# Freebirdgo/MapReduce_Rust

Measured on AMD Instinct MI355X. Metric: word-count input GB/s (whole node) at 1/2/4/8 MI355X + % of HBM roofline, higher is better.
Workload: dtype u8

## Files before the change

### mapreduce_rust_amd/csrc/k_keys.hip

```cpp
#include <algorithm>
#include <type_traits>

#include "mrg_device.h"
#include "mrg_internal.h"

namespace {

inline dim3 grid_for(uint64_t n, int b = 256) { return dim3((unsigned)((n + b - 1) / b)); }

template <int WG>
__device__ __forceinline__ uint64_t wg_append(unsigned long long *counter, bool pred, uint32_t *s_w,
                                              unsigned long long *s_base) {
    const uint64_t m = __ballot(pred);
    const uint32_t wv = threadIdx.x >> 6, lane = __lane_id();
    if (lane == 0) s_w[wv] = (uint32_t)__popcll(m);
    __syncthreads();
    if (threadIdx.x == 0) {
        uint32_t run = 0;
        for (int w = 0; w < WG / 64; ++w) {
            const uint32_t c = s_w[w];
            s_w[w] = run;
            run += c;
        }
        *s_base = run ? atomicAdd(counter, (unsigned long long)run) : 0ull;
// ... 387 lines not shown
    const uint64_t kbase = s_base;
    for (int pp = 0; pp < NP; ++pp) {
        const int i = min(pp * BA_WG + tid, (int)BA_CAP - 1);
        const BaKey k = s_key[i];
        const bool full = pp * BA_WG + tid < (int)BA_CAP && k.a != MRG_EMPTY_K0;
        const uint64_t m = __ballot(full);
        const uint64_t j = kbase + s_po[pp * BA_NW + wv] + (uint64_t)__popcll(m & mrg_lanemask_lt());
        if (full && j < A.kcap) {
            gk(A.out.k0)[j] = k.a;
            gk(A.out.k1)[j] = k.b;
            gk(A.out.cnt)[j] = s_cnt[i];
            gk(A.out.doc)[j] = IDX ? s_doc[i] : MRG_EMPTY_DOC;
            const uint32_t L = mrg_short_len(k.a, k.b);
            gk(A.out.len)[j] = L;
            gk(A.out.hoff)[j] = MRG_NO_HEAP;
            if (A.n_reduce) gk(A.out.part)[j] = (uint32_t)(mrg_siphash_short(k.a, k.b, L) % (uint64_t)A.n_reduce);
        }
    }
}

__global__ __launch_bounds__(1024) void k_stage_scatter(const uint8_t *stage, uint32_t table_off, uint32_t nops) {
    const StageOp *ops = reinterpret_cast<const StageOp *>(stage + table_off);
    for (uint32_t k = 0; k < nops; ++k) {
        const StageOp op = ops[k];
        uint8_t *dst = reinterpret_cast<uint8_t *>(op.dst);
        const bool fill = op.src == 0xFFFFFFFFu;
        if (((op.dst | op.n) & 3u) == 0u) {
            const uint32_t f4 = op.fill * 0x01010101u;
            const uint32_t *src = reinterpret_cast<const uint32_t *>(stage + (fill ? 0u : op.src));
            for (uint32_t i = threadIdx.x; i < op.n / 4u; i += blockDim.x)
                reinterpret_cast<uint32_t *>(dst)[i] = fill ? f4 : src[i];
// ... 354 lines not shown
    r.a = ks.k0[i];
    r.b = ks.k1[i];
    if (idx) {
        r.v = ks.doc[i];
        out[slot] = r;
        return;
    }
    for (uint64_t k = 0; k < nr; ++k) {
        const uint64_t c = cnt > vmax ? vmax : cnt;
        cnt -= c;
        r.v = (uint32_t)c;
        out[slot + k] = r;
    }
}

__global__ void k_make_sortrec(KeySet ks, uint64_t n, const uint32_t *doc_rank, SortRec *out, int carry) {
    const uint64_t i = (uint64_t)blockIdx.x * blockDim.x + threadIdx.x;
    if (i >= n) return;
    SortRec r;
    r.k0 = ks.k0[i];
    r.k1 = ks.k1[i];
    r.part = ks.part[i];
    r.doc = doc_rank ? doc_rank[ks.doc[i]] : 0u;
    r.idx = (uint32_t)i;
    r.pad = 0;
    if (carry) {
        const uint64_t c = ks.cnt[i];
        const uint32_t len = ks.len[i];
        r.doc = (uint32_t)c;
        r.pad = (len <= 16u ? len : 0xFFu) | ((uint32_t)(c >> 32) << 8);
    }
    out[i] = r;
// ... 76 lines not shown
}
void mrg_launch_export_count(KeySet ks, uint64_t n, uint32_t n_owners, unsigned long long *rec_cnt,
                             unsigned long long *heap_cnt, bool indexer, uint64_t vmax, hipStream_t s) {
    if (!n) return;
    hipLaunchKernelGGL(k_export_count, grid_for(n, EXP_WG), dim3(EXP_WG), 0, s, ks, n, n_owners, rec_cnt, heap_cnt,
                       indexer, vmax);
}
void mrg_launch_export_pack(KeySet ks, const uint8_t *heap, uint64_t n, uint32_t n_owners,
                            const uint64_t *rec_base, const uint64_t *heap_base, unsigned long long *rec_cur,
                            unsigned long long *heap_cur, XRec *out, uint8_t *out_heap, bool indexer, uint64_t vmax,
                            hipStream_t s) {
    if (!n) return;
    hipLaunchKernelGGL(k_export_pack, grid_for(n, EXP_WG), dim3(EXP_WG), 0, s, ks, heap, n, n_owners, rec_base,
                       heap_base, rec_cur, heap_cur, out, out_heap, indexer, vmax);
}
void mrg_launch_make_sortrec(KeySet ks, uint64_t n, const uint32_t *doc_rank, void *recs, hipStream_t s, bool carry) {
    if (!n) return;
    hipLaunchKernelGGL(k_make_sortrec, grid_for(n), dim3(256), 0, s, ks, n, doc_rank, (SortRec *)recs, carry ? 1 : 0);
}
void mrg_launch_wide_counts(const BucketArgs &a, uint64_t *cnt, uint64_t nseg, hipStream_t s) {
    hipLaunchKernelGGL(k_wide_counts, grid_for(nseg), dim3(256), 0, s, a, cnt);
}
void mrg_launch_wide_gather(const BucketArgs &a, const uint64_t *off, uint64_t nseg, uint32_t n_reduce, SortRec *out,
                            hipStream_t s) {
    hipLaunchKernelGGL(k_wide_gather, dim3((unsigned)nseg), dim3(256), 0, s, a, off, n_reduce, out);
}
void mrg_launch_wide_heads(const SortRec *r, uint64_t n, uint64_t *head, uint64_t *cv, hipStream_t s) {
    if (n) hipLaunchKernelGGL(k_wide_heads, grid_for(n), dim3(256), 0, s, r, n, head, cv);
}
void mrg_launch_wide_keys(const SortRec *r, uint64_t n, const uint64_t *head, const uint64_t *E, KeySet ks,
                          uint64_t *F, hipStream_t s) {
    if (n) hipLaunchKernelGGL(k_wide_keys, grid_for(n), dim3(256), 0, s, r, n, head, E, ks, F);
}
// ... 17 lines not shown
```

### mapreduce_rust_amd/csrc/k_map.hip

```cpp
#include "mrg_device.h"
#include "mrg_internal.h"
#include "mrg_split.h"

namespace {

constexpr int NW = MRG_MAP_WAVES;
constexpr int WG = 64 * NW;
constexpr int SEG = MRG_MAP_SEG;
constexpr int TILE = MRG_MAP_TILE;
constexpr int HALO = MRG_MAP_HALO;
constexpr int BEHIND = MRG_MAP_BEHIND;
constexpr int NSUB = MRG_MAP_NSUB;
constexpr int BLK = NSUB * TILE;
constexpr int WIN = BEHIND + TILE + HALO + 48;
constexpr int QCAP = TILE / 2 + 16;
constexpr int NMP = 64;
static_assert(TILE == 64 * SEG, "one segment per lane");
static_assert(WIN % 16 == 0, "16-byte window rows");
static_assert(NMP == TILE / SEG, "one mask pair per segment of the tile");
static_assert(16 * (1 + TILE / 16 + HALO / 16) <= WIN, "staged vectors fit the window row");
static_assert(BEHIND + (TILE - 1) + 31 + 20 <= WIN, "the 5-dword key read stays in the window row");
static_assert(BEHIND == 16 && HALO % 16 == 0 && HALO >= 64, "one 16-byte vector behind, whole halo vectors");
static_assert(QCAP >= TILE / 2 + 1, "the token queue holds every start of a tile");
static_assert(BLK == 2 * TILE && NSUB == 2, "A/B register sets hold two tiles per lane (v0, v1)");
// ... 1403 lines not shown
    lds_only_barrier();
    MRG_FT(1);
    if (tid < 64) {
        uint32_t run = 0;
        for (int b0 = 0; b0 < MRG_NBUCKET; b0 += 64) {
            const uint32_t v = s_hist[b0 + lane];
            const uint32_t inc = wave_incl_scan(v);
            s_hist[b0 + lane] = run + inc - v;
            run += lane_u32(inc, 63);
        }
        if (lane == 0) s_hist[MRG_NBUCKET] = run;
    }
    lds_only_barrier();
    MRG_FT(2);
    GAS uint32_t *foff = gp(A.foff) + (uint64_t)blockIdx.x * (MRG_NBUCKET + 1);
    for (int b = tid; b <= MRG_NBUCKET; b += WG) foff[b] = s_hist[b];
    const uint64_t reg = (uint64_t)blockIdx.x * CAP;
    for (int i = tid; i < CAP; i += WG) {
        const KeyPair k = s_key[i];
        if (k.a == MRG_EMPTY_K0) continue;
        const uint32_t d = IDX ? s_doc[i] : MRG_EMPTY_DOC;
        const uint32_t b = bucket_of(key_hash(k.a, k.b, d, A.hash_bits));
        const uint64_t pos2 = reg + s_hist[b] + s_rank[i];
        gp(A.fk0)[pos2] = k.a;
        gp(A.fk1)[pos2] = k.b;
        gp(A.fcnt)[pos2] = s_cnt[i];
        if (IDX) gp(A.fdoc)[pos2] = d;
    }
    }
    MRG_FT(3);
    uint32_t t = my_tokens, ttl = my_tail, t16 = my_tail16;
    for (int off = 32; off > 0; off >>= 1) {
        t += __shfl_down(t, off);
// ... 179 lines not shown
```

### mapreduce_rust_amd/csrc/k_sort.hip

```cpp
#include <algorithm>
#include <cstdlib>
#include <vector>

#include "mrg_device.h"
#include "mrg_internal.h"

namespace {

constexpr int BS = 256;
constexpr int IPT = 8;
constexpr int TILE = BS * IPT;

template <class T>
__device__ __forceinline__ T wave_incl_scan(T v) {
    const int lane = __lane_id();
    for (int o = 1; o < 64; o <<= 1) {
        const T u = __shfl_up(v, o);
        if (lane >= o) v += u;
    }
    return v;
}

template <class T>
__device__ __forceinline__ T block_excl_scan(T v, T *s_wave, T *total) {
// ... 196 lines not shown
    for (int q = 0; q < TR::NPASS; ++q) {
        if (!want[q]) continue;
        bool trivial = false;
        for (int d = 0; d < 256; ++d)
            if (h[q * 256 + d] == n) { trivial = true; break; }
        if (trivial) continue;
        hipLaunchKernelGGL(k_tile_hist<TR>, dim3(ntiles), dim3(BS), 0, s, a, n, q, cnt, ntiles);
        scan_rec<uint32_t>(cnt, cnt, (uint64_t)256 * ntiles, scantmp, s);
        hipLaunchKernelGGL(k_scatter<TR>, dim3(ntiles), dim3(BS), 0, s, a, b, n, q, cnt, ntiles);
        std::swap(a, b);
        if (passes_run) ++*passes_run;
    }
    return a;
}

constexpr int MSD_BITS = 20;
constexpr uint32_t MSD_NB = 1u << MSD_BITS;
constexpr int MSD_WG = 256;
constexpr uint32_t MSD_GRID = 1024;
constexpr uint32_t MSD_LCAP = 2048;
constexpr uint32_t MSD_SMALL = 64;
constexpr uint32_t MSD_SMALL_GRID = 2048;
constexpr uint32_t MSD_MAX_BIG = 16;

__device__ __forceinline__ uint32_t msd_bucket(const SortRec &r, uint32_t pbits) {
    if (pbits >= (uint32_t)MSD_BITS) return r.part >> (pbits - MSD_BITS);
    const uint32_t c0 = (uint32_t)(r.k0 >> 56), c1 = (uint32_t)(r.k0 >> 48) & 0xFFu, c2 = (uint32_t)(r.k0 >> 40) & 0xFFu;
    const uint32_t b0 = min(c0, 127u);
    const uint32_t b1 = b0 == 127u ? 127u : min(c1, 127u);
    const uint32_t b2 = b1 == 127u ? 127u : min(c2, 127u);
    const uint32_t code = (b0 << 14) | (b1 << 7) | b2;
    const uint32_t kb = MSD_BITS - pbits;
    return (r.part << kb) | (code >> (21 - kb));
}

__device__ __forceinline__ uint32_t uni_lane(uint32_t v, uint32_t j) {
    return (uint32_t)__builtin_amdgcn_readlane((int)v, (int)j);
}

__device__ __forceinline__ bool rec_less(const SortRec &a, const SortRec &b) {
    if (a.part != b.part) return a.part < b.part;
    if (a.k0 != b.k0) return a.k0 < b.k0;
    if (a.k1 != b.k1) return a.k1 < b.k1;
    if (a.doc != b.doc) return a.doc < b.doc;
    return a.idx < b.idx;
}

__global__ void k_msd_count(const SortRec *in, uint64_t n, uint32_t pbits, uint32_t *cnt, uint32_t *rank,
                            uint32_t *zero0, uint32_t *zero1, uint32_t *zero2) {
    const uint64_t i = (uint64_t)blockIdx.x * blockDim.x + threadIdx.x;
    if (i == 0) {
        *zero0 = 0;
        *zero1 = 0;
        *zero2 = 0;
    }
    if (i >= n) return;
    rank[i] = atomicAdd(&cnt[msd_bucket(in[i], pbits)], 1u);
}

__global__ void k_msd_scatter(const SortRec *in, SortRec *out, uint64_t n, uint32_t pbits, const uint32_t *off,
                              const uint32_t *rank) {
    const uint64_t i = (uint64_t)blockIdx.x * blockDim.x + threadIdx.x;
    if (i >= n) return;
    const SortRec r = in[i];
    out[off[msd_bucket(r, pbits)] + rank[i]] = r;
// ... 125 lines not shown
    void *ltmp;
};
static MsdTmp msd_tmp(void *tmp, uint64_t n) {
    MsdTmp t;
    t.cnt = (uint32_t *)tmp;
    t.off = t.cnt + (MSD_NB + 2);
    t.big = t.off + (MSD_NB + 2);
    t.list = t.big + (MSD_MAX_BIG + 2);
    t.list2 = t.list + (MSD_NB + 2);
    t.stmp = t.list2 + (MSD_NB + 2);
    t.rank = t.stmp + scan_tmp(MSD_NB + 1);
    t.ltmp = (void *)(((uintptr_t)(t.rank + n) + 255) & ~(uintptr_t)255);
    return t;
}

void mrg_msd_sort_launch(SortRec *a, SortRec *b, uint64_t n, uint32_t pbits, void *tmp, hipStream_t s,
                         uint32_t *h_nbig) {
    *h_nbig = 0;
    if (n <= 1) return;
    const MsdTmp t = msd_tmp(tmp, n);
    hipMemsetAsync(t.cnt, 0, sizeof(uint32_t) * (MSD_NB + 2), s);
    const unsigned g = (unsigned)((n + 255) / 256);
    hipLaunchKernelGGL(k_msd_count, dim3(g), dim3(256), 0, s, a, n, pbits, t.cnt, t.rank, t.big, t.list, t.list2);
    scan_rec<uint32_t>(t.cnt, t.off, MSD_NB + 1, t.stmp, s);
    hipLaunchKernelGGL(k_msd_scatter, dim3(g), dim3(256), 0, s, a, b, n, pbits, t.off, t.rank);
    uint32_t lcap = MSD_LCAP;
    if (const char *e = getenv("MRG_TEST_SORT_LCAP")) lcap = std::max<uint32_t>(1u, std::min<uint32_t>(MSD_LCAP, (uint32_t)atoi(e)));
    hipLaunchKernelGGL(k_msd_list, dim3(MSD_NB / 1024), dim3(1024), 0, s, t.off, std::min(MSD_SMALL, lcap), t.list, t.list2);
    const uint64_t nsmall = std::min<uint64_t>(n / 2, (uint64_t)MSD_SMALL_GRID * (MSD_WG / 64));
    hipLaunchKernelGGL(k_msd_leaf_small, dim3((unsigned)((nsmall + MSD_WG / 64 - 1) / (MSD_WG / 64))), dim3(MSD_WG), 0, s,
                       b, t.off, t.list);
    hipLaunchKernelGGL(k_msd_leaf, dim3(MSD_GRID), dim3(MSD_WG), 0, s, b, t.off, t.list2, lcap, t.big);
    hipMemcpyAsync(h_nbig, t.big, sizeof(uint32_t), hipMemcpyDeviceToHost, s);
}

SortRec *mrg_msd_sort_finish(SortRec *a, SortRec *b, uint64_t n, const SortPlan &plan, void *tmp, hipStream_t s,
                             uint32_t nb) {
    if (n <= 1) return a;
// ... 48 lines not shown
```

### mapreduce_rust_amd/csrc/mrg_internal.h

```cpp
#pragma once
#include <hip/hip_runtime.h>
#include <stddef.h>
#include <stdint.h>

#ifndef MRG_MAP_WAVES
#define MRG_MAP_WAVES 16
#endif
#define MRG_MAP_WG (64 * MRG_MAP_WAVES)
#define MRG_MAP_SEG 16
#define MRG_MAP_TILE (64 * MRG_MAP_SEG)
#define MRG_MAP_HALO 64
#define MRG_MAP_BEHIND 16
#define MRG_MAP_NSUB 2

#ifndef MRG_NBUCKET_LOG2
#define MRG_NBUCKET_LOG2 8
#endif
#define MRG_NBUCKET (1 << MRG_NBUCKET_LOG2)
#define MRG_BA_CAP 7680
#define MRG_TAIL_BYTES(idx) ((idx) ? 24u : 12u)

enum {
    CNT_REC = 0,
    CNT_LONG = 1,
// ... 133 lines not shown
    const uint32_t *monext;
    uint32_t mocap;
    const uint64_t *fk0, *fk1;
    const uint32_t *fcnt, *fdoc, *foff;
    uint32_t nreg, regcap;
    uint64_t *ok0, *ok1;
    uint32_t *ocnt, *odoc;
    uint64_t ocap;
    KeySet out;
    unsigned long long *counters;
    uint32_t hash_bits;
    uint32_t ablate;
    uint32_t nsub;
    uint64_t kcap;
    uint32_t n_reduce;
};
void mrg_launch_bucket_agg(const BucketArgs &a, bool indexer, bool count32, hipStream_t s);
struct SortRec;
void mrg_launch_wide_counts(const BucketArgs &a, uint64_t *cnt, uint64_t nseg, hipStream_t s);
void mrg_launch_wide_gather(const BucketArgs &a, const uint64_t *off, uint64_t nseg, uint32_t n_reduce, SortRec *out,
                            hipStream_t s);
void mrg_launch_wide_heads(const SortRec *r, uint64_t n, uint64_t *head, uint64_t *cv, hipStream_t s);
void mrg_launch_wide_keys(const SortRec *r, uint64_t n, const uint64_t *head, const uint64_t *E, KeySet ks,
                          uint64_t *F, hipStream_t s);
void mrg_launch_wide_cnt(const uint64_t *F, uint64_t runs, uint64_t n, const uint64_t *C, uint64_t ctot, KeySet ks,
                         hipStream_t s);
void mrg_launch_table_clear(const TableArgs &t, bool indexer, hipStream_t s);
void mrg_launch_table_insert(const TableArgs &t, const uint64_t *k0, const uint64_t *k1, const uint32_t *cnt32,
                             const uint32_t *doc, uint64_t n, bool indexer, hipStream_t s);
void mrg_launch_table_insert_x(const TableArgs &t, const XRec *x, uint64_t n, bool indexer, hipStream_t s);
// ... 7 lines not shown
void mrg_launch_long_emit(const uint32_t *rep, const uint64_t *cnt_in, const uint64_t *k0, const uint64_t *k1,
                          const uint32_t *flen, const uint64_t *hoff, const uint32_t *doc, uint64_t n,
                          unsigned long long *acc, KeySet out, unsigned long long *counter, bool indexer,
                          hipStream_t s);
void mrg_launch_x_split_long(const XRec *x, uint64_t n, const uint64_t *seg_rec_end, const uint64_t *seg_heap_base,
                             uint32_t n_segs, LongItems li, unsigned long long *counter, bool indexer, hipStream_t s);
void mrg_launch_l_split_long(const LRec *x, uint64_t n, const uint64_t *seg_rec_end, const uint64_t *seg_heap_base,
                             uint32_t n_segs, LongItems li, unsigned long long *counter, hipStream_t s);
void mrg_launch_export_count(KeySet ks, uint64_t n, uint32_t n_owners, unsigned long long *rec_cnt,
                             unsigned long long *heap_cnt, bool indexer, uint64_t vmax, hipStream_t s);
void mrg_launch_export_pack(KeySet ks, const uint8_t *heap, uint64_t n, uint32_t n_owners,
                            const uint64_t *rec_base, const uint64_t *heap_base, unsigned long long *rec_cur,
                            unsigned long long *heap_cur, XRec *out, uint8_t *out_heap, bool indexer, uint64_t vmax,
                            hipStream_t s);
void mrg_launch_make_sortrec(KeySet ks, uint64_t n, const uint32_t *doc_rank, void *recs, hipStream_t s,
                             bool carry = false);
void mrg_launch_fill_u32(uint32_t *p, uint32_t v, uint64_t n, hipStream_t s);
void mrg_launch_fill_u64(uint64_t *p, uint64_t v, uint64_t n, hipStream_t s);
void mrg_launch_iota_u32(uint32_t *p, uint64_t n, hipStream_t s);

uint64_t mrg_scan_tmp_elems(uint64_t n);
void mrg_scan_u64(const uint64_t *in, uint64_t *out, uint64_t n, uint64_t *tmp, hipStream_t s);
void mrg_scan_u32(const uint32_t *in, uint32_t *out, uint64_t n, uint32_t *tmp, hipStream_t s);
struct SortRec {
    uint64_t k0, k1;
    uint32_t part, doc;
    uint32_t idx, pad;
};
struct SortPlan {
    bool use_doc, use_k1, use_k0, use_part;
    uint32_t part_bytes;
    uint32_t doc_bytes;
};
uint64_t mrg_sort_tmp_bytes(uint64_t n);
SortRec *mrg_radix_sort(SortRec *recs, SortRec *alt, uint64_t n, const SortPlan &plan, void *tmp, hipStream_t s,
                        int *passes_run);
SortRec *mrg_msd_sort(SortRec *recs, SortRec *alt, uint64_t n, uint32_t pbits, const SortPlan &plan, void *tmp,
                      hipStream_t s, uint32_t *n_big, uint32_t *h_pinned);
void mrg_msd_sort_launch(SortRec *recs, SortRec *alt, uint64_t n, uint32_t pbits, void *tmp, hipStream_t s,
                         uint32_t *h_nbig);
SortRec *mrg_msd_sort_finish(SortRec *recs, SortRec *alt, uint64_t n, const SortPlan &plan, void *tmp, hipStream_t s,
                             uint32_t nb);
void mrg_radix_sort_u64(uint64_t *keys, uint32_t *vals, uint64_t *kv_tmp, uint64_t n, void *tmp, hipStream_t s);

struct FormatArgs {
    const SortRec *recs;
    uint64_t n;
    KeySet ks;
    const uint8_t *heap;
    uint64_t heap_bytes;
    uint32_t n_reduce;
    int drop_last;
    int indexer;
    int any_long;
    int carried;
// ... 185 lines not shown
```

### mapreduce_rust_amd/csrc/mrgpu.cpp

```cpp
#include <stdarg.h>
#include <stdio.h>
#include <string.h>
#include <sys/stat.h>

#include <rccl/rccl.h>

#include <fcntl.h>
#include <unistd.h>

#include <algorithm>
#include <atomic>
#include <chrono>
#include <condition_variable>
#include <map>
#include <memory>
#include <mutex>
#include <string>
#include <thread>
#include <unordered_map>
#include <vector>

#include "mrg_internal.h"
#include "mrgpu.h"

static_assert(sizeof(XRec) == MRG_XREC_BYTES, "exchange record layout (include/mrgpu.h)");

namespace {

thread_local std::string g_err;

struct MrgError {
    int code;
    std::string msg;
};

[[noreturn]] void raise(int code, const char *fmt, ...) {
    char buf[1024];
// ... 233 lines not shown
        p.put(leaf_pk);
        *this = WideRes{};
    }
};

struct Acc {
    bool on = false;
    bool dirty = false;
    bool seeded = false;
    AccTable T{};
    uint64_t n = 0;
    KeysBuf lng;
    uint64_t in_bytes = 0, tokens = 0, long_tokens = 0;
    uint32_t batches = 0, rehashes = 0;
    double ms_fold = 0.0;
};

}

struct mrg_ctx {
    int device = 0;
    hipStream_t own = nullptr, stream = nullptr;
    Pool pool;
    unsigned long long *d_cnt = nullptr;
    unsigned long long *h_cnt = nullptr;
    uint8_t *h_stage = nullptr;
    size_t stage_used = 0;
    uint8_t *d_stage = nullptr;
    std::vector<StageOp> pend;
    size_t pend_lo = 0;
// ... 28 lines not shown
    std::vector<uint64_t> exp_rec, exp_heap;
    uint64_t xrec_vmax = MRG_XREC_VMAX;
    uint8_t *d_out = nullptr;
    uint64_t out_cap = 0, out_bytes = 0;
    std::vector<uint64_t> part_off;
    bool reduced = false;
    uint8_t *d_final = nullptr;
    uint64_t final_cap = 0, final_bytes = 0;
    bool finalized = false;
    uint8_t *d_top = nullptr;
    uint64_t top_cap = 0, top_bytes = 0, top_lines = 0;
    bool topped = false;
    uint64_t top_info[8] = {};
    uint64_t top_pass_bytes[MRG_TOPK_DIGITS] = {};
    uint64_t extra_first = 0;
    mrg_stats st{};
    uint64_t enc_info[8] = {};
    double enc_ms[4] = {};
    hipEvent_t enc_ev[6] = {};
};

struct mrg_vocab {
    int device = 0;
    uint64_t n = 0, text_bytes = 0;
    void *block = nullptr;
    VocTable T{};
};

struct mrg_comm {
    ncclComm_t comm = nullptr;
// ... 80 lines not shown
    HIPCHK(hipMemcpyAsync(c->h_cnt, c->d_cnt, sizeof(unsigned long long) * CNT_N, hipMemcpyDeviceToHost, c->stream));
    sync(c);
}

void ev_rec(mrg_ctx *c, int i) {
    if (c->timing) HIPCHK(hipEventRecord(c->ev[i], c->stream));
}
double ev_ms(mrg_ctx *c, int a, int b) {
    if (!c->timing) return 0.0;
    float ms = 0;
    HIPCHK(hipEventSynchronize(c->ev[b]));
    HIPCHK(hipEventElapsedTime(&ms, c->ev[a], c->ev[b]));
    return ms;
}

void keys_release(mrg_ctx *c) {
    KeysBuf &k = c->keys;
    Pool &p = c->pool;
    p.put(k.ks.k0); p.put(k.ks.k1); p.put(k.ks.cnt); p.put(k.ks.hoff);
    p.put(k.ks.doc); p.put(k.ks.len); p.put(k.ks.part);
    p.put(k.heap);
    k = KeysBuf{};
}

void keysbuf_release(Pool &p, KeysBuf &k) {
    p.put(k.ks.k0); p.put(k.ks.k1); p.put(k.ks.cnt); p.put(k.ks.hoff);
    p.put(k.ks.doc); p.put(k.ks.len); p.put(k.ks.part);
    p.put(k.heap);
    k = KeysBuf{};
}

// ... 141 lines not shown
        p.put(fk0); p.put(fk1); p.put(fcnt); p.put(fdoc); p.put(foff);
        p.put(lstart); p.put(llen); p.put(ldoc); p.put(gbits);
        *this = MapBufs{};
    }
};

struct MapSteal;
void set_steal(mrg_ctx *c, MapArgs &A, MapBufs &M, const MapSteal &ms, uint64_t n_chunks);

struct AggLaunch {
    BucketArgs B{};
    uint64_t nlong = 0;
    bool c32 = false, live = false;
};

uint64_t agg_ocap(mrg_ctx *c) {
    uint64_t ocap = std::max<uint64_t>(c->ovf_hint, 1u << 20);
    if (const uint64_t t = env_u64("MRG_TEST_AGG_OCAP", 0)) ocap = t;
    return ocap;
}

AggLaunch agg_launch(mrg_ctx *c, const MapArgs &A, uint32_t nreg, uint32_t regcap, uint64_t ocap, uint32_t nsub,
                     uint64_t nlong, bool c32, bool zero) {
    Pool &p = c->pool;
    hipStream_t s = c->stream;
    const bool idx = is_idx(c);
    keys_reserve(c, (uint64_t)MRG_NBUCKET * std::max<uint32_t>(nsub, 1u) * MRG_BA_CAP + ocap + nlong + 1);
    AggLaunch L;
    BucketArgs &B = L.B;
    B.pool = A.pool; B.rbase = A.rbase; B.bcap = A.bcap; B.bcount = A.bcount;
    B.pool16 = A.pool16; B.rbase16 = A.rbase16; B.bcap16 = A.bcap16; B.bcount16 = A.bcount16;
    B.movf = A.ovf; B.monext = A.onext; B.mocap = A.ocap;
    B.fk0 = A.fk0; B.fk1 = A.fk1; B.fcnt = A.fcnt; B.fdoc = A.fdoc; B.foff = A.foff;
    B.nreg = nreg; B.regcap = regcap;
    B.ok0 = pget<uint64_t>(p, ocap); B.ok1 = pget<uint64_t>(p, ocap);
    B.ocnt = pget<uint32_t>(p, ocap); B.odoc = idx ? pget<uint32_t>(p, ocap) : nullptr;
    B.ocap = ocap;
    B.out = c->keys.ks;
    B.counters = c->d_cnt;
    B.hash_bits = hash_bits(c);
    B.ablate = getenv("MRG_AGG_ABLATE") ? (uint32_t)atoi(getenv("MRG_AGG_ABLATE")) : 0u;
    B.nsub = nsub;
    B.kcap = c->keys.cap;
    B.n_reduce = c->R;
    if (zero) {
        HIPCHK(hipMemsetAsync(&c->d_cnt[CNT_KEYS], 0, 8, s));
        HIPCHK(hipMemsetAsync(&c->d_cnt[CNT_OVF2], 0, 8, s));
    }
    mrg_launch_bucket_agg(B, idx, c32, s);
    L.nlong = nlong;
    L.c32 = c32;
    L.live = true;
    return L;
}

void agg_put(mrg_ctx *c, AggLaunch &L) {
    if (!L.live) return;
    Pool &p = c->pool;
    p.put(L.B.ok0); p.put(L.B.ok1); p.put(L.B.ocnt); p.put(L.B.odoc);
    L.live = false;
}

bool bucket_aggregate(mrg_ctx *c, const MapArgs &A, uint32_t nreg, uint32_t regcap, LongItems li,
                      AggLaunch *pre = nullptr) {
    if (nreg > 2048) raise(MRG_EINVAL, "internal: %u map workgroups exceed the aggregation's region table", nreg);
    const bool idx = is_idx(c);
    uint64_t ocap = agg_ocap(c);
    uint32_t agg_launches = 0;
    uint32_t nsub = c->agg_nsub;
    if (const uint64_t t = env_u64("MRG_TEST_AGG_NSUB", 0)) nsub = (uint32_t)t;
    const bool dirty = pre && pre->live;
    for (;;) {
        ++agg_launches;
        const bool c32 = c->h_cnt[CNT_TOKENS] < 0xFFFFFFFFull && nreg <= 512;
        AggLaunch L;
        if (pre && pre->live && agg_launches == 1 && pre->B.nsub == nsub && pre->B.ocap == ocap &&
            li.n <= pre->nlong &&
            pre->B.kcap >= (uint64_t)MRG_NBUCKET * std::max<uint32_t>(nsub, 1u) * MRG_BA_CAP + ocap + li.n + 1 &&
            pre->c32 == c32) {
            L = *pre;
            pre->live = false;
            c->st.spec_agg = 1;
        } else {
            if (pre && pre->live) c->st.spec_agg = 2;
            if (pre) agg_put(c, *pre);
            L = agg_launch(c, A, nreg, regcap, ocap, nsub, li.n, c32, agg_launches > 1 || dirty);
// ... 19 lines not shown
            agg_put(c, L);
            c->agg_nsub = 1;
            if (getenv("MRG_DEBUG")) fprintf(stderr, "[mrgpu] bucket agg: %llu overflow records -> wide\n", (unsigned long long)novf);
            return false;
        }
        if (novf > ocap) {
            agg_put(c, L);
            ocap = c->ovf_hint = novf + novf / 8 + 1024;
            continue;
        }
        if (novf) {
            ShortSrc src;
            src.k0 = B.ok0; src.k1 = B.ok1; src.cnt = B.ocnt; src.doc = B.odoc; src.n = novf;
            table_aggregate(c, src);
        }
        agg_put(c, L);
        c->st.overflow_keys = novf;
        c->st.agg_launches = agg_launches;
        c->spec_agg = !idx;
        c->spec_c32 = c32;
        c->st.agg_path = 1;
        c->wide_hint = false;
        {
            const uint64_t slots = idx ? 4096u : (c32 ? 6912u : 6112u);
            const uint64_t per = (uint64_t)MRG_NBUCKET * (slots * 5u / 6u);
            c->agg_nsub = (uint32_t)std::min<uint64_t>(16, std::max<uint64_t>(1, (c->h_cnt[CNT_KEYS] + per - 1) / per));
        }
        break;
    }
    const bool fresh = c->st.overflow_keys == 0 && li.n == 0;
    const uint64_t parted = std::min<uint64_t>(c->h_cnt[CNT_KEYS], c->keys.cap);
    long_aggregate(c, li);
    finish_keys(c, fresh, parted);
    return true;
}

uint32_t bytes_for(uint64_t maxval) {
    uint32_t b = 0;
    while (maxval) { ++b; maxval >>= 8; }
    return b;
}

void wide_aggregate_radix(mrg_ctx *c, const MapArgs &A, uint32_t nreg, uint32_t regcap, LongItems li) {
    Pool &p = c->pool;
    hipStream_t s = c->stream;
    BucketArgs B{};
    B.pool = A.pool; B.rbase = A.rbase; B.bcap = A.bcap; B.bcount = A.bcount;
    B.pool16 = A.pool16; B.rbase16 = A.rbase16; B.bcap16 = A.bcap16; B.bcount16 = A.bcount16;
// ... 1067 lines not shown
                throw;
            }
            relong = true;
        }
    }
    mrg_acc_launch_fold(A.T, b.ks, b.n, idx, &t.d_n[0], s);
    HIPCHK(hipGetLastError());
    uint64_t made = 0;
    HIPCHK(hipMemcpyAsync(&made, &t.d_n[0], 8, hipMemcpyDeviceToHost, s));
    sync(c);
    A.n += made;
    if (relong) {
        keysbuf_release(p, A.lng);
        A.lng = c->keys;
        c->keys = KeysBuf{};
    }
    A.dirty = true;
}

void acc_emit(mrg_ctx *c) {
    Acc &A = c->acc;
    if (!A.on || !A.dirty) return;
    Pool &p = c->pool;
    hipStream_t s = c->stream;
    const uint64_t n = A.n + A.lng.n;
    c->wide.release(p);
    keys_reserve(c, n + 1);
    KeysBuf &k = c->keys;
    HIPCHK(hipMemsetAsync(&c->d_cnt[CNT_KEYS], 0, sizeof(unsigned long long), s));
    if (A.T.cap) mrg_acc_launch_emit(A.T, is_idx(c), k.ks, A.n, &c->d_cnt[CNT_KEYS], s);
// ... 28 lines not shown
    need_job(c);
    if (c->doc_off.empty()) raise(MRG_EINVAL, "no input: call mrg_job_set_input first");
    Acc &A = c->acc;
    flush_stage(c);
    sync(c);
    c->stage_used = c->pend_lo = 0;
    if (!A.on) {
        if (c->keyed) {
            wide_densify(c, 0);
            A.on = A.seeded = true;
            A.in_bytes = c->st.input_bytes;
            A.tokens = c->st.tokens;
            A.long_tokens = c->st.long_tokens;
            KeysBuf b = c->keys;
            c->keys = KeysBuf{};
            c->keyed = false;
            try {
                acc_fold(c, b);
            } catch (...) {
                acc_release(c);
                c->mapped = false;
                throw;
            }
        }
        A.on = true;
    }
    const mrg_stats st0 = c->st;
    const bool had = A.seeded || A.batches;
    try {
        job_map(c);
        wide_densify(c, 0);
        KeysBuf b = c->keys;
        c->keys = KeysBuf{};
        c->keyed = false;
        acc_fold(c, b);
        ev_rec(c, 7);
        A.ms_fold = ev_ms(c, 3, 7);
    } catch (...) {
        keys_release(c);
        c->wide.release(c->pool);
        c->keyed = false;
        c->st = st0;
        c->mapped = had;
        c->reduced = false;
        A.dirty = true;
        throw;
    }
    A.in_bytes += c->st.input_bytes;
// ... 54 lines not shown
    const bool idx = is_idx(c);
    SortPlan plan{};
    plan.use_part = R > 1;
    plan.part_bytes = bytes_for(R - 1);
    plan.use_k0 = plan.use_k1 = true;
    plan.use_doc = idx;
    plan.doc_bytes = idx ? bytes_for(c->names.size() - 1) : 0;
    return plan;
}

SortRec *sort_keys(mrg_ctx *c, KeySet ks, uint32_t R, const uint32_t *d_rank, SortRec *a, SortRec *b, void *stmp,
                   bool defer = false, bool carry = false) {
    const uint64_t n = c->keys.n;
    mrg_launch_make_sortrec(ks, n, d_rank, a, c->stream, carry);
    check_sort_n(n, "key sort");
    const uint32_t pbits = R > 1 ? 32u - (uint32_t)__builtin_clz(R - 1u) : 0u;
    uint32_t *h_nbig = (uint32_t *)&c->h_cnt[CNT_N];
    if (defer) {
        mrg_msd_sort_launch(a, b, n, pbits, stmp, c->stream, h_nbig);
        return n <= 1 ? a : b;
    }
    uint32_t n_big = 0;
    return mrg_msd_sort(a, b, n, pbits, sort_plan(c, R), stmp, c->stream, &n_big, h_nbig);
}

FormatArgs format_args(mrg_ctx *c, const SortRec *recs, KeySet ks, uint32_t R, int drop_last, const DocRank &dr,
                       bool carried = false) {
    FormatArgs f{};
    f.carried = carried ? 1 : 0;
    f.recs = recs;
    f.n = c->keys.n;
// ... 51 lines not shown
}

void job_reduce(mrg_ctx *c) {
    need_job(c);
    if (!c->mapped) raise(MRG_EINVAL, "nothing to reduce: call mrg_job_map or mrg_job_import first");
    acc_emit(c);
    if (c->wide.ready) {
        wide_reduce(c);
        return;
    }
    Pool &p = c->pool;
    hipStream_t s = c->stream;
    const uint64_t n = c->keys.n;
    DocRank dr = doc_ranks(c);
    ev_rec(c, 4);
    SortRec *a = pget<SortRec>(p, n), *b = pget<SortRec>(p, n);
    void *stmp = p.get(mrg_sort_tmp_bytes(n));
    SortRec *sorted = a;
    const bool presorted = c->keys.sorted && !c->keys.any_long && !is_idx(c);
    const bool defer = !presorted && !(c->extra_first && n);
    const bool carry = !is_idx(c) && !c->extra_first;
    if (presorted) mrg_launch_make_sortrec(c->keys.ks, n, nullptr, a, s, carry);
    else sorted = sort_keys(c, c->keys.ks, c->R, dr.rank, a, b, stmp, defer, carry);
    if (c->extra_first && n) {
        if (c->keys.any_long) mrg_launch_fix_runs(sorted, n, c->keys.ks, c->keys.heap, s);
        mrg_launch_add_first(sorted, c->keys.ks, c->extra_first, s);
    }
    ev_rec(c, 5);
    const FormatArgs f = format_args(c, sorted, c->keys.ks, c->R, compat_drop_last(c), dr, carry);
    c->part_off.assign(c->R + 1, 0);
    c->out_bytes = mrg_format(f, p, &c->d_out, &c->out_cap, c->part_off.data(), s);
    const uint32_t n_big = *(const uint32_t *)&c->h_cnt[CNT_N];
    if (defer && n > 1 && n_big) {
        sorted = mrg_msd_sort_finish(a, b, n, sort_plan(c, c->R), stmp, s, n_big);
        const FormatArgs f2 = format_args(c, sorted, c->keys.ks, c->R, compat_drop_last(c), dr, carry);
        c->out_bytes = mrg_format(f2, p, &c->d_out, &c->out_cap, c->part_off.data(), s);
    }
    ev_rec(c, 6);
    HIPCHK(hipGetLastError());
    p.put(a); p.put(b); p.put(stmp);
    dr.release(p);
    c->st.ms_sort = ev_ms(c, 4, 5);
    c->st.ms_format = ev_ms(c, 5, 6);
    c->st.output_bytes = c->out_bytes;
    c->reduced = true;
}

void job_final(mrg_ctx *c) {
    need_job(c);
    if (!c->mapped) raise(MRG_EINVAL, "no keys: call mrg_job_map or mrg_job_import first");
    acc_emit(c);
    wide_densify(c, 0);
    Pool &p = c->pool;
    hipStream_t s = c->stream;
    const uint64_t n = c->keys.n;
// ... 804 lines not shown
}

int mrg_close(mrg_ctx *c) {
    return guard([&] {
        if (!c) return;
        (void)hipSetDevice(c->device);
        (void)hipStreamSynchronize(c->stream);
        for (auto &e : c->ev) (void)hipEventDestroy(e);
        for (auto &e : c->enc_ev)
            if (e) (void)hipEventDestroy(e);
        (void)hipFree(c->d_cnt);
        (void)hipHostFree(c->h_cnt);
        if (c->h_stage) (void)hipHostFree(c->h_stage);
        if (c->d_stage) (void)hipFree(c->d_stage);
        if (c->own) (void)hipStreamDestroy(c->own);
        delete c;
    });
}

int mrg_set_stream(mrg_ctx *c, void *hip_stream) {
    return guard([&] {
        if (!c) raise(MRG_EINVAL, "null context");
        sync(c);
        c->stream = hip_stream ? (hipStream_t)hip_stream : c->own;
    });
}

int mrg_set_timing(mrg_ctx *c, int enable) {
    return guard([&] {
        if (!c) raise(MRG_EINVAL, "null context");
// ... 160 lines not shown
        if (!v) raise(MRG_EINVAL, "null vocabulary");
        if (cap < v->text_bytes) raise(MRG_EINVAL, "destination too small (%llu < %llu)", (unsigned long long)cap,
                                       (unsigned long long)v->text_bytes);
        if (!v->text_bytes) return;
        if (!h_dst) raise(MRG_EINVAL, "null argument");
        HIPCHK(hipSetDevice(v->device));
        HIPCHK(hipMemcpy(h_dst, v->T.text, v->text_bytes, hipMemcpyDeviceToHost));
    });
}

void mrg_vocab_free(mrg_vocab *v) { vocab_destroy(v); }

int mrg_vocab_encode(mrg_ctx *c, const mrg_vocab *v, const uint8_t *d_bytes, const uint64_t *h_doc_off, uint32_t n_docs,
                     uint32_t *d_ids, uint64_t cap_ids, uint64_t *h_tok_off) {
    return guard([&] { vocab_encode(c, v, d_bytes, h_doc_off, n_docs, d_ids, cap_ids, h_tok_off); });
}

int mrg_encode_info(mrg_ctx *c, uint64_t *h_info, double *h_ms) {
    return guard([&] {
        if (!c) raise(MRG_EINVAL, "null context");
        if (h_info) memcpy(h_info, c->enc_info, sizeof c->enc_info);
        if (h_ms) memcpy(h_ms, c->enc_ms, sizeof c->enc_ms);
    });
}

int mrg_map_text(mrg_ctx *c, const uint8_t *h_bytes, size_t n, uint32_t n_reduce, uint8_t **h_out,
                 uint64_t *h_part_off) {
    return guard([&] {
        if (!c || !h_out || !h_part_off || (n && !h_bytes)) raise(MRG_EINVAL, "null argument");
        if (n_reduce == 0) raise(MRG_EINVAL, "n_reduce must be > 0");
// ... 852 lines not shown
```

### mapreduce_rust_amd/native.py

```python
import ctypes as C
import os

_HERE = os.path.dirname(os.path.abspath(__file__))

APP_WC = 0
APP_INDEXER = 1
FLAG_NO_COMPAT_DROP_LAST = 0x1
FLAG_FINAL_TXT = 0x2
FLAG_STREAM = 0x4
XREC_BYTES = 24
ABI_VERSION = 6
ID_UNK = 0xFFFFFFFF

OK, EINVAL, EUTF8, EHIP, ENOMEM, EIO, ECOMM = 0, -1, -2, -3, -4, -5, -6
_CODES = {EINVAL: "EINVAL", EUTF8: "EUTF8", EHIP: "EHIP", ENOMEM: "ENOMEM", EIO: "EIO", ECOMM: "ECOMM"}
COMM_ID_BYTES = 128


def debug_hash_bits(n):
    return (n & 0xFF) << 8


def flag_top(k):
    return (k & 0xFFFF) << 16
# ... 285 lines not shown
    def import_(self, d_rec, n_rec, d_heap, heap_bytes, seg_recs=None, seg_heap=None):
        if seg_recs is None:
            _check(load().mrg_job_import(self.h, d_rec, n_rec, d_heap, heap_bytes, None, None, 0))
        else:
            _check(load().mrg_job_import(self.h, d_rec, n_rec, d_heap, heap_bytes, _u64arr(seg_recs),
                                         _u64arr(seg_heap), len(seg_recs)))

    def shuffle(self, comm):
        _check(load().mrg_job_shuffle(self.h, comm.h))

    def reduce(self):
        n = C.c_uint64()
        _check(load().mrg_job_reduce(self.h, C.byref(n)))
        return n.value

    def output(self):
        d = _vp()
        off = (C.c_uint64 * (self.n_reduce + 1))()
        _check(load().mrg_job_output(self.h, C.byref(d), off))
        return d.value, list(off)

    def copy_output(self):
        _, off = self.output()
        buf = C.create_string_buffer(max(off[-1], 1))
        _check(load().mrg_job_copy_output(self.h, buf, off[-1]))
        return buf.raw[:off[-1]], off

    def copy_output_to(self, host_ptr, n):
        _check(load().mrg_job_copy_output(self.h, C.c_void_p(host_ptr), n))

# ... 174 lines not shown
```

Before: 1334.

## Emit sort records and MSD bucket counts directly from bucket aggregation

The bucket-aggregate kernel now writes 32-byte SortRec entries and atomically bumps MSD bucket histogram counters as it emits keys. Only the tail of keys added after aggregation (long keys) goes through make_sortrec and count. At reduce time the prepared records skip the separate make_sortrec pass, memset and count kernel. This removes a full read/write pass over the key set before sorting. In exchange, aggregation does extra global stores and atomics, the sort buffer is held across phases, and the ABL_CONST guard adds a compile-time ablation switch in map.

```diff
diff --git a/mapreduce_rust_amd/csrc/k_keys.hip b/mapreduce_rust_amd/csrc/k_keys.hip
--- a/mapreduce_rust_amd/csrc/k_keys.hip
+++ b/mapreduce_rust_amd/csrc/k_keys.hip
@@ -3,6 +3,7 @@
 
 #include "mrg_device.h"
 #include "mrg_internal.h"
+#include "mrg_msd.h"
 
 namespace {
 
@@ -425,7 +426,27 @@
             const uint32_t L = mrg_short_len(k.a, k.b);
             gk(A.out.len)[j] = L;
             gk(A.out.hoff)[j] = MRG_NO_HEAP;
-            if (A.n_reduce) gk(A.out.part)[j] = (uint32_t)(mrg_siphash_short(k.a, k.b, L) % (uint64_t)A.n_reduce);
+            uint32_t part = 0;
+            if (A.n_reduce) gk(A.out.part)[j] = part = (uint32_t)(mrg_siphash_short(k.a, k.b, L) % (uint64_t)A.n_reduce);
+            if constexpr (!IDX && C32) {
+                if (A.srec) {
+                    static_assert(sizeof(SortRec) == 32 && offsetof(SortRec, part) == 16 && offsetof(SortRec, doc) == 20 &&
+                                  offsetof(SortRec, idx) == 24 && offsetof(SortRec, pad) == 28, "record words below");
+                    GASK uint64_t *o = reinterpret_cast<GASK uint64_t *>(gk(A.srec) + j);
+                    o[0] = k.a;
+                    o[1] = k.b;
+                    o[2] = (uint64_t)part | ((uint64_t)s_cnt[i] << 32);
+                    o[3] = (uint64_t)(uint32_t)j | ((uint64_t)L << 32);
+                    gk(A.srank)[j] = atomicAdd(&A.scnt[mrg_msd_bucket(part, k.a, A.pbits)], 1u);
+                }
+            }
+        }
+    }
+    if constexpr (!IDX && C32) {
+        if (A.srec && blockIdx.x == 0 && tid == 0) {
+            *A.sz0 = 0;
+            *A.sz1 = 0;
+            *A.sz2 = 0;
         }
     }
 }
@@ -810,8 +831,8 @@
     }
 }
 
-__global__ void k_make_sortrec(KeySet ks, uint64_t n, const uint32_t *doc_rank, SortRec *out, int carry) {
-    const uint64_t i = (uint64_t)blockIdx.x * blockDim.x + threadIdx.x;
+__global__ void k_make_sortrec(KeySet ks, uint64_t first, uint64_t n, const uint32_t *doc_rank, SortRec *out, int carry) {
+    const uint64_t i = first + (uint64_t)blockIdx.x * blockDim.x + threadIdx.x;
     if (i >= n) return;
     SortRec r;
     r.k0 = ks.k0[i];
@@ -918,9 +939,11 @@
     hipLaunchKernelGGL(k_export_pack, grid_for(n, EXP_WG), dim3(EXP_WG), 0, s, ks, heap, n, n_owners, rec_base,
                        heap_base, rec_cur, heap_cur, out, out_heap, indexer, vmax);
 }
-void mrg_launch_make_sortrec(KeySet ks, uint64_t n, const uint32_t *doc_rank, void *recs, hipStream_t s, bool carry) {
-    if (!n) return;
-    hipLaunchKernelGGL(k_make_sortrec, grid_for(n), dim3(256), 0, s, ks, n, doc_rank, (SortRec *)recs, carry ? 1 : 0);
+void mrg_launch_make_sortrec(KeySet ks, uint64_t n, const uint32_t *doc_rank, void *recs, hipStream_t s, bool carry,
+                             uint64_t first) {
+    if (first >= n) return;
+    hipLaunchKernelGGL(k_make_sortrec, grid_for(n - first), dim3(256), 0, s, ks, first, n, doc_rank, (SortRec *)recs,
+                       carry ? 1 : 0);
 }
 void mrg_launch_wide_counts(const BucketArgs &a, uint64_t *cnt, uint64_t nseg, hipStream_t s) {
     hipLaunchKernelGGL(k_wide_counts, grid_for(nseg), dim3(256), 0, s, a, cnt);
diff --git a/mapreduce_rust_amd/csrc/k_map.hip b/mapreduce_rust_amd/csrc/k_map.hip
--- a/mapreduce_rust_amd/csrc/k_map.hip
+++ b/mapreduce_rust_amd/csrc/k_map.hip
@@ -1441,9 +1441,9 @@
     lds_only_barrier();
     MRG_FT(2);
     GAS uint32_t *foff = gp(A.foff) + (uint64_t)blockIdx.x * (MRG_NBUCKET + 1);
-    for (int b = tid; b <= MRG_NBUCKET; b += WG) foff[b] = s_hist[b];
+    for (int b = tid; b <= MRG_NBUCKET; b += WG) foff[b] = (MRG_MAP_ABL_CONST & 0x40000u) ? 0u : s_hist[b];
     const uint64_t reg = (uint64_t)blockIdx.x * CAP;
-    for (int i = tid; i < CAP; i += WG) {
+    for (int i = tid; i < ((MRG_MAP_ABL_CONST & 0x40000u) ? 0 : CAP); i += WG) {
         const KeyPair k = s_key[i];
         if (k.a == MRG_EMPTY_K0) continue;
         const uint32_t d = IDX ? s_doc[i] : MRG_EMPTY_DOC;
diff --git a/mapreduce_rust_amd/csrc/k_sort.hip b/mapreduce_rust_amd/csrc/k_sort.hip
--- a/mapreduce_rust_amd/csrc/k_sort.hip
+++ b/mapreduce_rust_amd/csrc/k_sort.hip
@@ -4,6 +4,7 @@
 
 #include "mrg_device.h"
 #include "mrg_internal.h"
+#include "mrg_msd.h"
 
 namespace {
 
@@ -234,7 +235,7 @@
     return a;
 }
 
-constexpr int MSD_BITS = 20;
+constexpr int MSD_BITS = MRG_MSD_BITS;
 constexpr uint32_t MSD_NB = 1u << MSD_BITS;
 constexpr int MSD_WG = 256;
 constexpr uint32_t MSD_GRID = 1024;
@@ -244,14 +245,7 @@
 constexpr uint32_t MSD_MAX_BIG = 16;
 
 __device__ __forceinline__ uint32_t msd_bucket(const SortRec &r, uint32_t pbits) {
-    if (pbits >= (uint32_t)MSD_BITS) return r.part >> (pbits - MSD_BITS);
-    const uint32_t c0 = (uint32_t)(r.k0 >> 56), c1 = (uint32_t)(r.k0 >> 48) & 0xFFu, c2 = (uint32_t)(r.k0 >> 40) & 0xFFu;
-    const uint32_t b0 = min(c0, 127u);
-    const uint32_t b1 = b0 == 127u ? 127u : min(c1, 127u);
-    const uint32_t b2 = b1 == 127u ? 127u : min(c2, 127u);
-    const uint32_t code = (b0 << 14) | (b1 << 7) | b2;
-    const uint32_t kb = MSD_BITS - pbits;
-    return (r.part << kb) | (code >> (21 - kb));
+    return mrg_msd_bucket(r.part, r.k0, pbits);
 }
 
 __device__ __forceinline__ uint32_t uni_lane(uint32_t v, uint32_t j) {
@@ -266,9 +260,9 @@
     return a.idx < b.idx;
 }
 
-__global__ void k_msd_count(const SortRec *in, uint64_t n, uint32_t pbits, uint32_t *cnt, uint32_t *rank,
+__global__ void k_msd_count(const SortRec *in, uint64_t first, uint64_t n, uint32_t pbits, uint32_t *cnt, uint32_t *rank,
                             uint32_t *zero0, uint32_t *zero1, uint32_t *zero2) {
-    const uint64_t i = (uint64_t)blockIdx.x * blockDim.x + threadIdx.x;
+    const uint64_t i = first + (uint64_t)blockIdx.x * blockDim.x + threadIdx.x;
     if (i == 0) {
         *zero0 = 0;
         *zero1 = 0;
@@ -424,14 +418,29 @@
     return t;
 }
 
+MsdPrep mrg_msd_prep(void *tmp, hipStream_t s) {
+    const MsdTmp t = msd_tmp(tmp, 0);
+    hipMemsetAsync(t.cnt, 0, sizeof(uint32_t) * (MSD_NB + 2), s);
+    return MsdPrep{t.cnt, t.rank, t.big, t.list, t.list2};
+}
+
+void mrg_msd_count_range(const SortRec *a, uint64_t first, uint64_t n, uint32_t pbits, void *tmp, hipStream_t s) {
+    if (first >= n) return;
+    const MsdTmp t = msd_tmp(tmp, n);
+    hipLaunchKernelGGL(k_msd_count, dim3((unsigned)((n - first + 255) / 256)), dim3(256), 0, s, a, first, n, pbits, t.cnt,
+                       t.rank, t.big, t.list, t.list2);
+}
+
 void mrg_msd_sort_launch(SortRec *a, SortRec *b, uint64_t n, uint32_t pbits, void *tmp, hipStream_t s,
-                         uint32_t *h_nbig) {
+                         uint32_t *h_nbig, bool counted) {
     *h_nbig = 0;
     if (n <= 1) return;
     const MsdTmp t = msd_tmp(tmp, n);
-    hipMemsetAsync(t.cnt, 0, sizeof(uint32_t) * (MSD_NB + 2), s);
     const unsigned g = (unsigned)((n + 255) / 256);
-    hipLaunchKernelGGL(k_msd_count, dim3(g), dim3(256), 0, s, a, n, pbits, t.cnt, t.rank, t.big, t.list, t.list2);
+    if (!counted) {
+        hipMemsetAsync(t.cnt, 0, sizeof(uint32_t) * (MSD_NB + 2), s);
+        hipLaunchKernelGGL(k_msd_count, dim3(g), dim3(256), 0, s, a, (uint64_t)0, n, pbits, t.cnt, t.rank, t.big, t.list, t.list2);
+    }
     scan_rec<uint32_t>(t.cnt, t.off, MSD_NB + 1, t.stmp, s);
     hipLaunchKernelGGL(k_msd_scatter, dim3(g), dim3(256), 0, s, a, b, n, pbits, t.off, t.rank);
     uint32_t lcap = MSD_LCAP;
diff --git a/mapreduce_rust_amd/csrc/mrg_internal.h b/mapreduce_rust_amd/csrc/mrg_internal.h
--- a/mapreduce_rust_amd/csrc/mrg_internal.h
+++ b/mapreduce_rust_amd/csrc/mrg_internal.h
@@ -171,6 +171,9 @@
     uint32_t nsub;
     uint64_t kcap;
     uint32_t n_reduce;
+    struct SortRec *srec;
+    uint32_t *scnt, *srank, *sz0, *sz1, *sz2;
+    uint32_t pbits;
 };
 void mrg_launch_bucket_agg(const BucketArgs &a, bool indexer, bool count32, hipStream_t s);
 struct SortRec;
@@ -208,7 +211,7 @@
                             unsigned long long *heap_cur, XRec *out, uint8_t *out_heap, bool indexer, uint64_t vmax,
                             hipStream_t s);
 void mrg_launch_make_sortrec(KeySet ks, uint64_t n, const uint32_t *doc_rank, void *recs, hipStream_t s,
-                             bool carry = false);
+                             bool carry = false, uint64_t first = 0);
 void mrg_launch_fill_u32(uint32_t *p, uint32_t v, uint64_t n, hipStream_t s);
 void mrg_launch_fill_u64(uint64_t *p, uint64_t v, uint64_t n, hipStream_t s);
 void mrg_launch_iota_u32(uint32_t *p, uint64_t n, hipStream_t s);
@@ -232,7 +235,12 @@
 SortRec *mrg_msd_sort(SortRec *recs, SortRec *alt, uint64_t n, uint32_t pbits, const SortPlan &plan, void *tmp,
                       hipStream_t s, uint32_t *n_big, uint32_t *h_pinned);
 void mrg_msd_sort_launch(SortRec *recs, SortRec *alt, uint64_t n, uint32_t pbits, void *tmp, hipStream_t s,
-                         uint32_t *h_nbig);
+                         uint32_t *h_nbig, bool counted = false);
+struct MsdPrep {
+    uint32_t *cnt, *rank, *z0, *z1, *z2;
+};
+MsdPrep mrg_msd_prep(void *tmp, hipStream_t s);
+void mrg_msd_count_range(const SortRec *recs, uint64_t first, uint64_t n, uint32_t pbits, void *tmp, hipStream_t s);
 SortRec *mrg_msd_sort_finish(SortRec *recs, SortRec *alt, uint64_t n, const SortPlan &plan, void *tmp, hipStream_t s,
                              uint32_t nb);
 void mrg_radix_sort_u64(uint64_t *keys, uint32_t *vals, uint64_t *kv_tmp, uint64_t n, void *tmp, hipStream_t s);
diff --git a/mapreduce_rust_amd/csrc/mrg_msd.h b/mapreduce_rust_amd/csrc/mrg_msd.h
--- /dev/null
+++ b/mapreduce_rust_amd/csrc/mrg_msd.h
@@ -0,0 +1,16 @@
+#pragma once
+#include <hip/hip_runtime.h>
+#include <stdint.h>
+
+constexpr int MRG_MSD_BITS = 20;
+
+__device__ __forceinline__ uint32_t mrg_msd_bucket(uint32_t part, uint64_t k0, uint32_t pbits) {
+    if (pbits >= (uint32_t)MRG_MSD_BITS) return part >> (pbits - MRG_MSD_BITS);
+    const uint32_t c0 = (uint32_t)(k0 >> 56), c1 = (uint32_t)(k0 >> 48) & 0xFFu, c2 = (uint32_t)(k0 >> 40) & 0xFFu;
+    const uint32_t b0 = min(c0, 127u);
+    const uint32_t b1 = b0 == 127u ? 127u : min(c1, 127u);
+    const uint32_t b2 = b1 == 127u ? 127u : min(c2, 127u);
+    const uint32_t code = (b0 << 14) | (b1 << 7) | b2;
+    const uint32_t kb = MRG_MSD_BITS - pbits;
+    return (part << kb) | (code >> (21 - kb));
+}
diff --git a/mapreduce_rust_amd/csrc/mrgpu.cpp b/mapreduce_rust_amd/csrc/mrgpu.cpp
--- a/mapreduce_rust_amd/csrc/mrgpu.cpp
+++ b/mapreduce_rust_amd/csrc/mrgpu.cpp
@@ -21,6 +21,7 @@
 #include <vector>
 
 #include "mrg_internal.h"
+#include "mrg_msd.h"
 #include "mrgpu.h"
 
 static_assert(sizeof(XRec) == MRG_XREC_BYTES, "exchange record layout (include/mrgpu.h)");
@@ -284,6 +285,14 @@
     uint64_t in_bytes = 0, tokens = 0, long_tokens = 0;
     uint32_t batches = 0, rehashes = 0;
     double ms_fold = 0.0;
+};
+
+struct SortPrep {
+    SortRec *recs = nullptr;
+    void *tmp = nullptr;
+    uint64_t cap = 0, n_agg = 0, n = 0;
+    uint32_t pbits = 0;
+    bool valid = false;
 };
 
 }
@@ -342,6 +351,8 @@
     uint64_t top_info[8] = {};
     uint64_t top_pass_bytes[MRG_TOPK_DIGITS] = {};
     uint64_t extra_first = 0;
+    SortPrep prep;
+    uint64_t reduce_info[4] = {};
     mrg_stats st{};
     uint64_t enc_info[8] = {};
     double enc_ms[4] = {};
@@ -452,7 +463,13 @@
     return ms;
 }
 
+void prep_drop(mrg_ctx *c) {
+    c->pool.put(c->prep.recs);
+    c->prep = SortPrep{};
+}
+
 void keys_release(mrg_ctx *c) {
+    prep_drop(c);
     KeysBuf &k = c->keys;
     Pool &p = c->pool;
     p.put(k.ks.k0); p.put(k.ks.k1); p.put(k.ks.cnt); p.put(k.ks.hoff);
@@ -624,6 +641,8 @@
     bool c32 = false, live = false;
 };
 
+uint32_t sort_pbits(uint32_t R) { return R > 1 ? 32u - (uint32_t)__builtin_clz(R - 1u) : 0u; }
+
 uint64_t agg_ocap(mrg_ctx *c) {
     uint64_t ocap = std::max<uint64_t>(c->ovf_hint, 1u << 20);
     if (const uint64_t t = env_u64("MRG_TEST_AGG_OCAP", 0)) ocap = t;
@@ -653,6 +672,18 @@
     B.nsub = nsub;
     B.kcap = c->keys.cap;
     B.n_reduce = c->R;
+    const uint32_t pbits = sort_pbits(c->R);
+    if (!idx && c32 && pbits < (uint32_t)MRG_MSD_BITS && !c->acc.on && c->keys.cap <= 0x7FFFFFFFull) {
+        SortPrep &P = c->prep;
+        P.cap = c->keys.cap;
+        const uint64_t rbytes = (sizeof(SortRec) * P.cap + 255) & ~255ull;
+        P.recs = (SortRec *)p.get(rbytes + mrg_sort_tmp_bytes(P.cap));
+        P.tmp = (uint8_t *)P.recs + rbytes;
+        P.pbits = pbits;
+        const MsdPrep m = mrg_msd_prep(P.tmp, s);
+        B.srec = P.recs; B.scnt = m.cnt; B.srank = m.rank; B.sz0 = m.z0; B.sz1 = m.z1; B.sz2 = m.z2;
+        B.pbits = pbits;
+    }
     if (zero) {
         HIPCHK(hipMemsetAsync(&c->d_cnt[CNT_KEYS], 0, 8, s));
         HIPCHK(hipMemsetAsync(&c->d_cnt[CNT_OVF2], 0, 8, s));
@@ -680,6 +711,7 @@
     uint32_t nsub = c->agg_nsub;
     if (const uint64_t t = env_u64("MRG_TEST_AGG_NSUB", 0)) nsub = (uint32_t)t;
     const bool dirty = pre && pre->live;
+    bool armed = false;
     for (;;) {
         ++agg_launches;
         const bool c32 = c->h_cnt[CNT_TOKENS] < 0xFFFFFFFFull && nreg <= 512;
@@ -729,6 +761,7 @@
             src.k0 = B.ok0; src.k1 = B.ok1; src.cnt = B.ocnt; src.doc = B.odoc; src.n = novf;
             table_aggregate(c, src);
         }
+        armed = B.srec != nullptr && B.srec == c->prep.recs;
         agg_put(c, L);
         c->st.overflow_keys = novf;
         c->st.agg_launches = agg_launches;
@@ -747,6 +780,15 @@
     const uint64_t parted = std::min<uint64_t>(c->h_cnt[CNT_KEYS], c->keys.cap);
     long_aggregate(c, li);
     finish_keys(c, fresh, parted);
+    if (armed) {
+        SortPrep &P = c->prep;
+        const uint64_t n = c->keys.n;
+        mrg_launch_make_sortrec(c->keys.ks, n, nullptr, P.recs, c->stream, true, parted);
+        mrg_msd_count_range(P.recs, parted, n, P.pbits, P.tmp, c->stream);
+        P.n_agg = parted;
+        P.n = n;
+        P.valid = true;
+    }
     return true;
 }
 
@@ -1844,6 +1886,7 @@
         keysbuf_release(p, A.lng);
         A.lng = c->keys;
         c->keys = KeysBuf{};
+        prep_drop(c);
     }
     A.dirty = true;
 }
@@ -1902,6 +1945,7 @@
             A.long_tokens = c->st.long_tokens;
             KeysBuf b = c->keys;
             c->keys = KeysBuf{};
+            prep_drop(c);
             c->keyed = false;
             try {
                 acc_fold(c, b);
@@ -1920,6 +1964,7 @@
         wide_densify(c, 0);
         KeysBuf b = c->keys;
         c->keys = KeysBuf{};
+        prep_drop(c);
         c->keyed = false;
         acc_fold(c, b);
         ev_rec(c, 7);
@@ -2004,7 +2049,7 @@
     const uint64_t n = c->keys.n;
     mrg_launch_make_sortrec(ks, n, d_rank, a, c->stream, carry);
     check_sort_n(n, "key sort");
-    const uint32_t pbits = R > 1 ? 32u - (uint32_t)__builtin_clz(R - 1u) : 0u;
+    const uint32_t pbits = sort_pbits(R);
     uint32_t *h_nbig = (uint32_t *)&c->h_cnt[CNT_N];
     if (defer) {
         mrg_msd_sort_launch(a, b, n, pbits, stmp, c->stream, h_nbig);
@@ -2086,14 +2131,33 @@
     const uint64_t n = c->keys.n;
     DocRank dr = doc_ranks(c);
     ev_rec(c, 4);
-    SortRec *a = pget<SortRec>(p, n), *b = pget<SortRec>(p, n);
-    void *stmp = p.get(mrg_sort_tmp_bytes(n));
+    const bool presorted = c->keys.sorted && !c->keys.any_long && !is_idx(c);
+    SortPrep &P = c->prep;
+    const bool prepared = P.valid && P.n == n && n > 1 && n <= P.cap && !presorted && !c->extra_first && !is_idx(c) &&
+                          !c->acc.on && P.pbits == sort_pbits(c->R);
+    c->reduce_info[0] = prepared ? 1 : 0;
+    c->reduce_info[1] = prepared ? P.n_agg : 0;
+    c->reduce_info[2] = n;
+    SortRec *a = nullptr;
+    void *stmp = nullptr;
+    if (prepared) {
+        a = P.recs;
+        stmp = P.tmp;
+        P = SortPrep{};
+    } else {
+        prep_drop(c);
+        a = pget<SortRec>(p, n);
+        stmp = p.get(mrg_sort_tmp_bytes(n));
+    }
+    SortRec *b = pget<SortRec>(p, n);
     SortRec *sorted = a;
-    const bool presorted = c->keys.sorted && !c->keys.any_long && !is_idx(c);
     const bool defer = !presorted && !(c->extra_first && n);
     const bool carry = !is_idx(c) && !c->extra_first;
     if (presorted) mrg_launch_make_sortrec(c->keys.ks, n, nullptr, a, s, carry);
-    else sorted = sort_keys(c, c->keys.ks, c->R, dr.rank, a, b, stmp, defer, carry);
+    else if (prepared) {
+        mrg_msd_sort_launch(a, b, n, sort_pbits(c->R), stmp, s, (uint32_t *)&c->h_cnt[CNT_N], true);
+        sorted = b;
+    } else sorted = sort_keys(c, c->keys.ks, c->R, dr.rank, a, b, stmp, defer, carry);
     if (c->extra_first && n) {
         if (c->keys.any_long) mrg_launch_fix_runs(sorted, n, c->keys.ks, c->keys.heap, s);
         mrg_launch_add_first(sorted, c->keys.ks, c->extra_first, s);
@@ -2110,7 +2174,8 @@
     }
     ev_rec(c, 6);
     HIPCHK(hipGetLastError());
-    p.put(a); p.put(b); p.put(stmp);
+    p.put(a); p.put(b);
+    if (!prepared) p.put(stmp);
     dr.release(p);
     c->st.ms_sort = ev_ms(c, 4, 5);
     c->st.ms_format = ev_ms(c, 5, 6);
@@ -2945,6 +3010,7 @@
         if (c->h_stage) (void)hipHostFree(c->h_stage);
         if (c->d_stage) (void)hipFree(c->d_stage);
         if (c->own) (void)hipStreamDestroy(c->own);
+        prep_drop(c);
         delete c;
     });
 }
@@ -3135,6 +3201,13 @@
 int mrg_vocab_encode(mrg_ctx *c, const mrg_vocab *v, const uint8_t *d_bytes, const uint64_t *h_doc_off, uint32_t n_docs,
                      uint32_t *d_ids, uint64_t cap_ids, uint64_t *h_tok_off) {
     return guard([&] { vocab_encode(c, v, d_bytes, h_doc_off, n_docs, d_ids, cap_ids, h_tok_off); });
+}
+
+int mrg_test_reduce_info(mrg_ctx *c, uint64_t *h_info) {
+    return guard([&] {
+        if (!c || !h_info) raise(MRG_EINVAL, "null argument");
+        memcpy(h_info, c->reduce_info, sizeof c->reduce_info);
+    });
 }
 
 int mrg_encode_info(mrg_ctx *c, uint64_t *h_info, double *h_ms) {
diff --git a/mapreduce_rust_amd/native.py b/mapreduce_rust_amd/native.py
--- a/mapreduce_rust_amd/native.py
+++ b/mapreduce_rust_amd/native.py
@@ -323,6 +323,14 @@
         _check(load().mrg_job_reduce(self.h, C.byref(n)))
         return n.value
 
+    def reduce_info(self):
+        f = load().mrg_test_reduce_info
+        f.restype = C.c_int
+        f.argtypes = [_vp, _u64p]
+        info = (C.c_uint64 * 4)()
+        _check(f(self.h, info))
+        return {"prepared": bool(info[0]), "n_agg": info[1], "n": info[2]}
+
     def output(self):
         d = _vp()
         off = (C.c_uint64 * (self.n_reduce + 1))()
```

Result: no change. 1344 (median of 6 runs) (+0.7%).
